# jeong0982/gkr

Hardware: AMD Instinct MI355X
Metric: BN254-Fr sumcheck field-ops/sec @ 2^20 vars (higher is better)
Workload: dtype u32x8

## Files before the change

gkr_amd/csrc/kernels.h:

```cpp
#pragma once
#include <hip/hip_runtime.h>
#include <stddef.h>
#include <stdint.h>

#include "fr32.h"

namespace gkr {

constexpr uint32_t kMaxBlocksPerTable = 2048;
constexpr uint32_t kMaxLayerBlocks = 2048;

struct MlePartial {
    Acc<9> lo, hi;
    uint32_t dep, pad;
};

struct LayerBatch {
    uint32_t batch;
    uint32_t pstride;
    size_t tstride, wstride;
};
inline LayerBatch single_layer() { return LayerBatch{1u, 0u, 0, 0}; }

struct LayerPartial {
    Acc<9> c0, g1, c2;
    uint32_t pad;
};

struct MleHostRec {
    Fr c0, c1;
    uint32_t dep, seq;
    uint32_t pad[14];
};
struct LayerHostRec {
    Fr c0, g1, c2;
    uint32_t seq;
    uint32_t pad[7];
};
static_assert(sizeof(MleHostRec) == 128 && sizeof(LayerHostRec) == 128, "hand-off records are one 128-byte line");

constexpr int kProdMaxJ = 3;
constexpr int kProdRecValues = 72;
struct ProdPassRec {
    Fr v[kProdRecValues];
    uint32_t seq;
    uint32_t pad[7];
};
static_assert(sizeof(ProdPassRec) == kProdRecValues * 32 + 32, "product-pass record layout");
constexpr uint32_t kProdTile = 8, kProdTileWide = 32;
inline uint32_t prod_pass_tile(uint32_t S) { return S >= 1024u ? kProdTileWide : kProdTile; }
inline uint32_t prod_pass_blocks(uint32_t S) { return S <= kProdTile ? 1u : S / prod_pass_tile(S); }
inline uint32_t prod_pass_max_blocks(uint32_t k) {
    uint32_t m = 1;
    for (uint32_t l = 0; l < k; ++l) m = prod_pass_blocks(1u << l) > m ? prod_pass_blocks(1u << l) : m;
    return m;
}
inline size_t prod_pass_scratch_values(uint32_t k) { return ((size_t)prod_pass_max_blocks(k) + 64u) * kProdRecValues; }
constexpr uint32_t kProdFuseBlocks = 64;
constexpr uint32_t kProdFoldMinM = 17;
size_t prod_fold_plan_bytes();
void launch_prod_pass(Fr* W, Fr* X, Fr* Y, uint32_t m_in, uint32_t jp, const Fr* weights, uint32_t J, Fr* partials, uint32_t wstride,
                      ProdPassRec* rec, uint32_t ticket, uint32_t batch, hipStream_t s, uint32_t* arrivals = nullptr, void* fold_plans = nullptr,
                      Fr* tail = nullptr, uint32_t tail_stride = 0);
void launch_prod_c_setup(const Fr* Wb, uint32_t jp, const Fr* weights, const Fr* A, const Fr* M, Fr* X, Fr* Y, uint32_t k, uint32_t wstride,
                         uint32_t batch, hipStream_t s);

constexpr uint32_t kSmallFoldQuarter = 2048;
void launch_mle_fold_sum_small(const Fr* src, size_t src_stride, Fr* dst, size_t dst_stride, uint32_t q, uint32_t batch,
                               const FixedMul* rtab, MleHostRec* host_rec, uint32_t ticket, hipStream_t s);
void launch_mle_round_reduce(const MlePartial* partials, uint32_t nblk, uint32_t batch, MleHostRec* host_rec,
                             uint32_t ticket, hipStream_t s);

struct MleSubPartial {
    Acc<9> sum;
    uint32_t dep, pad[2];
};
constexpr int kMlePassMaxRounds = 5;
constexpr int kMleMaxSub = 1 << kMlePassMaxRounds;
struct MleHostRecSub {
    Fr sums[kMleMaxSub];
    uint32_t dep, seq;
    uint32_t pad[14];
};
static_assert(sizeof(MleHostRecSub) == 1088, "hand-off record layout");
struct MlePublish {
    MleHostRecSub* rec = nullptr;
    uint32_t* arrivals = nullptr;
    uint32_t ticket = 0, jout = 0;
};
constexpr uint32_t kSmallPassEntries = 512;
uint32_t mle_pass_blocks(uint32_t items, uint32_t jout, uint32_t batch);
uint32_t mle_multifold_blocks(uint32_t S, uint32_t jout, uint32_t batch);
bool mle_multifold_uses_mfma(uint32_t S, uint32_t nblk);
constexpr int kMlePass0Stream = 2;
constexpr uint64_t kMlePass0DeepMinPartials = 2u * 12u * 256u * 4u;
void launch_mle_sub_sums(const Fr* tables, size_t stride, uint32_t len, uint32_t batch, uint32_t nblk, MleSubPartial* partials,
                         hipStream_t s, const MlePublish* publish = nullptr);
void launch_mle_sub_reduce(const MleSubPartial* partials, uint32_t nblk, uint32_t jout, uint32_t batch, MleHostRecSub* host_rec,
                           uint32_t ticket, hipStream_t s);
size_t mle_fold_plan_bytes();
void launch_mle_fold_plan(int jin, const Fr* weights, void* plans, uint32_t batch, hipStream_t s, uint32_t threads = 0);
void launch_mle_multifold(int jin, const Fr* src, size_t src_stride, Fr* dst, size_t dst_stride, uint32_t S, uint32_t batch,
                          uint32_t nblk, const Fr* weights, const void* plans, MleSubPartial* partials, hipStream_t s,
                          const MlePublish* publish = nullptr);
void launch_mle_pass_hash_lanes(const MleHostRecSub* rec, uint32_t count, uint32_t J, uint32_t round0, uint32_t n_out, bool final_pass,
                                bool first_pass, const Fr* cts, uint32_t* dep_last, Fr* weights, Fr* out_coeffs, uint32_t* out_len, Fr* out_r,
                                hipStream_t s);
void launch_mle_multifold_small(int jin, const Fr* src, size_t src_stride, Fr* dst, size_t dst_stride, uint32_t S, uint32_t jout,
                                uint32_t batch, const Fr* weights, MleHostRecSub* host_rec, uint32_t ticket, hipStream_t s, Fr* tail = nullptr, uint32_t tail_stride = 0,
                                uint32_t planes = 1, uint32_t plane_stride = 0);
constexpr uint32_t kMleFold2Planes = 8;
uint32_t mle_multifold2_partials(uint32_t S);
uint32_t mle_multifold2_tiles(uint32_t S);
void launch_mle_fine_sums(const MleSubPartial* partials, uint32_t nblk, const Fr* weights, uint32_t batch, MleHostRecSub* host_rec, uint32_t ticket,
                          hipStream_t s);
void launch_mle_copy_weights(const Fr* src, Fr* dst, uint32_t batch, hipStream_t s);
void launch_mle_multifold2(const Fr* src, size_t src_stride, Fr* dst, size_t dst_stride, uint32_t S, uint32_t batch, const void* plans, const Fr* w2,
                           MleSubPartial* partials, hipStream_t s);
void launch_layer_round_reduce(const LayerPartial* partials, uint32_t nblk, LayerHostRec* host_rec, uint32_t ticket,
                               LayerBatch lb, hipStream_t s);
void launch_fold_small(Fr* W, uint32_t hw, const FixedMul* rtab, LayerBatch lb, hipStream_t s);
struct GateSpan {
    uint64_t base, count;
};
uint32_t gate_lists_lds_blocks(uint64_t gates, uint32_t k);
size_t gate_lists_lds_scratch_words(uint64_t gates, uint32_t k);
inline size_t gate_list_words(uint64_t gates) { return 2 * (size_t)gates + 1; }
struct GateSegs {
    uint32_t shift = 0;
    uint32_t runs = 0;
    uint32_t run_base = 0;
    uint32_t bound = 0;
    uint32_t half_bound = 0;
    uint32_t groups = 0;
    uint32_t nb = 0;
    uint64_t packed_half = 0;
    uint32_t* words = nullptr;
    uint2* items() const { return reinterpret_cast<uint2*>(words); }
    uint32_t* order() const { return words + 2 * (size_t)bound; }
    uint32_t* bucket_begin() const { return order() + bound; }
    uint32_t* group_len() const { return bucket_begin() + 2 * (size_t)nb + 2; }
    uint32_t* group_off() const { return group_len() + 2 * (size_t)groups; }
    uint32_t* packed() const { return group_off() + 2 * (size_t)groups + 2; }
};
uint32_t gate_seg_shift(GateSpan span, uint32_t k_i, uint32_t k);
size_t gate_segs_words(GateSpan span, uint32_t k_i, uint32_t k);
size_t gate_segs_scratch_words(GateSpan span, uint32_t k_i, uint32_t k);
size_t gate_seg_partial_elems(GateSpan span, uint32_t k_i, uint32_t k);
void launch_gate_lists(GateSpan span, uint32_t k_i, uint32_t k, const uint8_t* gate_type, const uint32_t* left, const uint32_t* right,
                       uint32_t* counts, uint32_t* offsets, uint32_t* cursor, uint32_t* block_sums, uint32_t* list, uint32_t* bad,
                       uint32_t* lds_scratch, GateSegs* segs, uint32_t* seg_scratch, hipStream_t s);
struct GateSet {
    const uint32_t* offsets;
    const uint32_t* cursor;
    const uint32_t* list;
    const uint32_t* plan;
    const uint8_t* gate_type;
    const uint32_t* left;
    const uint32_t* right;
    uint64_t pad;
};
static_assert(sizeof(GateSet) == 64, "one cache line per proof");
void launch_gate_uv(GateSpan span, uint32_t k_i, uint32_t k, const uint32_t* offsets, const uint32_t* cursor, const uint32_t* list,
                    const Fr* e_hi, const Fr* e_lo_mont, uint32_t kl, const Fr* W, Fr* U, Fr* V, LayerBatch lb, const GateSegs* segs,
                    Fr* partials, hipStream_t s, const GateSet* sets = nullptr);
struct CPhaseFuse {
    const Fr* Wb = nullptr;
    const Fr* weights = nullptr;
    Fr* X = nullptr;
    Fr* Y = nullptr;
    uint32_t jp = 0;
};
bool launch_gate_rows(GateSpan span, uint32_t k_i, uint32_t k, const uint32_t* offsets, const uint32_t* cursor, const uint32_t* list,
                      const Fr* e_hi, const Fr* e_lo_mont, uint32_t kl, const Fr* eq_mont, Fr* A_row, Fr* M_row, LayerBatch lb,
                      const GateSegs* segs, Fr* partials, hipStream_t s, const CPhaseFuse* fuse = nullptr, const GateSet* sets = nullptr);
void launch_fill_table(Fr* table, size_t count, uint64_t seed, hipStream_t s);
void launch_fill_shard(Fr* shard_table, size_t count, uint32_t lp, uint32_t shard, uint64_t seed, hipStream_t s);
// ... 206 lines not shown
```

gkr_amd/csrc/kernels.hip:

```cpp
#include <hip/hip_runtime.h>
#include <stdlib.h>

#include <atomic>

#include "kernels.h"
#include "options.h"
#include "dev_util.h"
#include "gate_seg.h"
#include "mfma_fold.h"
#include "mfma_cross.h"
#include "mimc7.h"

namespace gkr {


__device__ __forceinline__ uint64_t mix64(uint64_t z) {
    z = (z ^ (z >> 30)) * 0xBF58476D1CE4E5B9ULL;
    z = (z ^ (z >> 27)) * 0x94D049BB133111EBULL;
    return z ^ (z >> 31);
}

__global__ void k_fill_table(Fr* table, size_t count, uint64_t seed) {
    for (size_t i = blockIdx.x * (size_t)blockDim.x + threadIdx.x; i < count; i += (size_t)gridDim.x * blockDim.x) {
        Fr f;
// ... 254 lines not shown
        : "v"(x.x), "v"(x.y), "v"(x.z), "v"(x.w)
        : "vcc");
}

template <int U, int PPW>
__global__ void __launch_bounds__(256) k_mle_sub_sums_stream(const Fr* __restrict__ tables, size_t table_stride, uint32_t chunk, uint32_t nblk,
                                                             MleSubPartial* __restrict__ partials) {
    static_assert(U >= 2 && (U & (U - 1)) == 0, "two sets of U / 2 loads");
    constexpr int H = U / 2;
    const uint32_t lane = threadIdx.x & 63u;
    const uint32_t wave = __builtin_amdgcn_readfirstlane(threadIdx.x >> 6);
    const uint32_t p0 = (blockIdx.x * 4u + wave) * (uint32_t)PPW;
    const uint32_t rpp = chunk / (32u * U);
    const mf_v4u* src = reinterpret_cast<const mf_v4u*>(tables + (size_t)blockIdx.y * table_stride + (size_t)p0 * chunk) + lane;
    MleSubPartial* out = partials + (size_t)blockIdx.y * nblk + p0;

    mf_v4u xa[H], xb[H];
    uint32_t acc[5] = {0u, 0u, 0u, 0u, 0u}, diff = 0u;
    auto load_set = [&](mf_v4u (&x)[H], const mf_v4u* p) {
#pragma unroll
        for (int u = 0; u < H; ++u) x[u] = __builtin_nontemporal_load(p + (size_t)u * 64u);
    };
    auto add_set = [&](const mf_v4u (&x)[H]) {
#pragma unroll
        for (int u = 0; u < H; ++u) {
            half_acc_add(acc, x[u]);
            const mf_v4u v = x[u];
            diff |= (v.x ^ (uint32_t)__builtin_amdgcn_mov_dpp((int)v.x, 0x4E, 0xF, 0xF, true)) |
                    (v.y ^ (uint32_t)__builtin_amdgcn_mov_dpp((int)v.y, 0x4E, 0xF, 0xF, true)) |
                    (v.z ^ (uint32_t)__builtin_amdgcn_mov_dpp((int)v.z, 0x4E, 0xF, 0xF, true)) |
                    (v.w ^ (uint32_t)__builtin_amdgcn_mov_dpp((int)v.w, 0x4E, 0xF, 0xF, true));
        }
    };
    auto finish = [&](MleSubPartial* p) {
        const bool odd = (lane & 1u) != 0u;
        Acc<9> s;
#pragma unroll
        for (int i = 0; i < 4; ++i) {
            s.l[i] = odd ? 0u : acc[i];
            s.l[4 + i] = odd ? acc[i] : (i == 0 ? acc[4] : 0u);
        }
        s.l[8] = odd ? acc[4] : 0u;
        s = wave_sum(s);
        const uint32_t dep = __any(diff != 0u) ? 1u : 0u;
        if (lane == 0) {
            p->sum = s;
            p->dep = dep;
        }
    };

#pragma unroll
    for (int u = 0; u < H; ++u) {
        xa[u] = __builtin_nontemporal_load(src + (size_t)u * 64u);
        __builtin_amdgcn_sched_barrier(0);
    }
#pragma unroll
    for (int u = 0; u < H; ++u) {
        xb[u] = __builtin_nontemporal_load(src + (size_t)(H + u) * 64u);
        __builtin_amdgcn_sched_barrier(0);
    }
    src += (size_t)U * 64u;
    [[maybe_unused]] uint32_t left = rpp;
    for (uint32_t r = (uint32_t)PPW * rpp - 1u; r != 0u; --r) {
        add_set(xa);
        load_set(xa, src);
        __builtin_amdgcn_sched_barrier(0);
        add_set(xb);
        load_set(xb, src + (size_t)H * 64u);
        __builtin_amdgcn_sched_barrier(0);
        src += (size_t)U * 64u;
        if constexpr (PPW > 1) {
            if (--left == 0u) {
                finish(out++);
#pragma unroll
                for (int i = 0; i < 5; ++i) acc[i] = 0u;
                diff = 0u;
                left = rpp;
            }
        }
    }
    add_set(xa);
    add_set(xb);
    finish(out);
}

template <int JIN>
__global__ void __launch_bounds__(256) k_mle_multifold(const Fr* __restrict__ src, size_t src_stride, Fr* __restrict__ dst,
                                                       size_t dst_stride, uint32_t S, const Fr* __restrict__ weights,
                                                       MleSubPartial* __restrict__ partials, MlePublish pub) {
    __shared__ Acc<9> smem[4];
    const Fr* s = src + (size_t)blockIdx.y * src_stride;
    Fr* d = dst + (size_t)blockIdx.y * dst_stride;
    const Fr* w = weights + (size_t)blockIdx.y * kMleMaxSub;
    const uint32_t chunk = S / gridDim.x;
    const uint32_t begin = blockIdx.x * chunk, end = begin + chunk;
    Acc<9> acc[1] = {acc_zero<9>()};
    for (uint32_t i = begin + threadIdx.x; i < end; i += blockDim.x) {
        const Fr y = multifold_entry<JIN>(s, S, i, w);
        store_fr(d + i, y);
        acc_add_fr(acc[0], y);
    }
    block_sum<9, 1>(acc, smem);
    if (threadIdx.x == 0) {
        MleSubPartial* p = partials + (size_t)blockIdx.y * gridDim.x + blockIdx.x;
        p->sum = acc[0];
        p->dep = 0;
    }
    if (pub.arrivals) mle_publish_from_last_block(partials, pub);
}

template <int JIN>
__global__ void __launch_bounds__(1024) k_mle_fold_plan(const Fr* __restrict__ weights, MfmaFoldPlan* __restrict__ plans) {
    __shared__ __attribute__((aligned(16))) unsigned char digits[32 * 32 * (1 << JIN)];
    mfma_plan_block<JIN>(weights + (size_t)blockIdx.x * kMleMaxSub, plans + blockIdx.x, digits);
}

template <int JIN>
__global__ void __launch_bounds__(256) k_mle_multifold_mfma(const Fr* __restrict__ src, size_t src_stride, Fr* __restrict__ dst,
                                                            size_t dst_stride, uint32_t S, const MfmaFoldPlan* __restrict__ plans,
                                                            MleSubPartial* __restrict__ partials, MlePublish pub) {
    __shared__ Acc<9> smem[4];
    __shared__ __attribute__((aligned(16))) unsigned char digits[JIN > 2 ? 32 * 32 * (1 << JIN) : 16];
    const Fr* s = src + (size_t)blockIdx.y * src_stride;
    Fr* d = dst + (size_t)blockIdx.y * dst_stride;
    const uint32_t chunk = S / gridDim.x;
    const uint32_t begin = blockIdx.x * chunk;
    Acc<9> acc[1] = {acc_zero<9>()};
    mfma_multifold_block<JIN>(s, d, S, plans + blockIdx.y, begin, begin + chunk, blockIdx.x * 5u + blockIdx.y * 3u, acc[0], digits);
    block_sum<9, 1>(acc, smem);
    if (threadIdx.x == 0) {
        MleSubPartial* p = partials + (size_t)blockIdx.y * gridDim.x + blockIdx.x;
        p->sum = acc[0];
        p->dep = 0;
    }
    if (pub.arrivals) mle_publish_from_last_block(partials, pub);
}


__global__ void __launch_bounds__(256) k_mle_fine_sums(const MleSubPartial* __restrict__ partials, uint32_t nblk, const Fr* __restrict__ weights,
                                                       MleHostRecSub* __restrict__ host_rec, uint32_t ticket) {
    __shared__ Fr s_w[kMleMaxSub];
    __shared__ Fr s_p[kMleMaxSub][8];
    const uint32_t t = threadIdx.x, q = t >> 5, c = t & 31u, run = nblk >> 10;
    const MleSubPartial* p = partials + (size_t)blockIdx.x * nblk;
    s_w[t >> 3].l[t & 7u] = reinterpret_cast<const uint32_t*>(weights + (size_t)blockIdx.x * kMleMaxSub)[t];
    static_assert(kMleMaxSub * 8 == 256, "one word of the weights per thread");
    __syncthreads();
    Lazy17 dot = lazy_zero();
    for (uint32_t k = 0; k < 4u; ++k) {
        const uint32_t b = q + 8u * k;
        Acc<10> f = acc_zero<10>();
        for (uint32_t i = 0; i < run; ++i) acc_add_acc(f, p[(size_t)(b * 32u + c) * run + i].sum);
        lazy_mac_v(dot, acc_reduce(f), s_w[b]);
    }
    s_p[c][q] = lazy_reduce(dot);
    __syncthreads();
    MleHostRecSub* r = host_rec + blockIdx.x;
    if (t < kMleMaxSub) {
        Acc<9> tot = acc_zero<9>();
        for (uint32_t k = 0; k < 8u; ++k) acc_add_fr(tot, s_p[t][k]);
        r->sums[t] = acc_reduce(tot);
    }
    __syncthreads();
    if (t == 0) __hip_atomic_store(&r->seq, ticket, __ATOMIC_RELEASE, __HIP_MEMORY_SCOPE_SYSTEM);
}

// ... 1848 lines not shown
    static std::atomic<uint64_t> attr_set{0};
    int dev = 0;
    (void)hipGetDevice(&dev);
    if (LDS_T && !((attr_set.load(std::memory_order_relaxed) >> (dev & 63)) & 1u)) {
        if (hipFuncSetAttribute(reinterpret_cast<const void*>(&k_seg_pass<ROWS, LDS_T>), hipFuncAttributeMaxDynamicSharedMemorySize, 160 * 1024) != hipSuccess) {
            (void)hipGetLastError();
            launch_seg_pass_t<ROWS, false>(g, k, e_lo_mont, T, X, Y, lb, s);
            return;
        }
        attr_set.fetch_or((uint64_t)1 << (dev & 63), std::memory_order_relaxed);
    }
    const uint32_t blocks = LDS_T ? device_cus() : 4 * device_cus();
    hipLaunchKernelGGL((k_seg_pass<ROWS, LDS_T>), dim3(blocks, lb.batch), dim3(LDS_T ? 1024 : 256), lds, s, g.items(), g.order(), g.bucket_begin(),
                       g.nb, g.groups, g.group_len(), g.group_off(), g.packed(), e_lo_mont, g.shift, T, tlen,
                       (uint32_t)lb.wstride, X, Y, g.half_bound);
}
static void launch_seg_pass(bool rows, const GateSegs& g, uint32_t k, const Fr* e_lo_mont, const Fr* T, Fr* X, Fr* Y, LayerBatch lb, hipStream_t s) {
    const bool no_lds = opt(OPT_gate_segments_no_lds) != 0;
    const bool lds_t = !no_lds && ((size_t)sizeof(Fr) << k) <= 128 * 1024;
    if (rows)
        lds_t ? launch_seg_pass_t<true, true>(g, k, e_lo_mont, T, X, Y, lb, s) : launch_seg_pass_t<true, false>(g, k, e_lo_mont, T, X, Y, lb, s);
    else
        lds_t ? launch_seg_pass_t<false, true>(g, k, e_lo_mont, T, X, Y, lb, s) : launch_seg_pass_t<false, false>(g, k, e_lo_mont, T, X, Y, lb, s);
}

void launch_exclusive_scan(const uint32_t* in, uint32_t* out, uint32_t* block_sums, size_t n, hipStream_t s) {
    const uint32_t sblocks = (uint32_t)((n + kScanPerBlock - 1) / kScanPerBlock);
    hipLaunchKernelGGL(k_scan_blocks, dim3(sblocks), dim3(256), 0, s, in, out, block_sums, n);
    hipLaunchKernelGGL(k_scan_sums, dim3(1), dim3(1024), 0, s, block_sums, sblocks);
    hipLaunchKernelGGL(k_scan_add, dim3(sblocks), dim3(256), 0, s, out, (uint32_t*)nullptr, block_sums, n);
}

static uint32_t bucket_threads(uint64_t gates, uint32_t k) { return (gates >> k) > 64u ? 256u : 64u; }

void launch_gate_uv(GateSpan span, uint32_t k_i, uint32_t k, const uint32_t* offsets, const uint32_t* cursor, const uint32_t* list,
                    const Fr* e_hi, const Fr* e_lo_mont, uint32_t kl, const Fr* W, Fr* U, Fr* V, LayerBatch lb, const GateSegs* segs,
                    Fr* partials, hipStream_t s, const GateSet* sets) {
    if (segs && segs->shift && partials && !sets) {
        Fr *X = partials, *Y = partials + (size_t)segs->half_bound * lb.batch;
        launch_seg_pass(false, *segs, k, e_lo_mont, W, X, Y, lb, s);
        hipLaunchKernelGGL(k_seg_combine, dim3(((1u << k) + 1u) / 2u, lb.batch), dim3(64), 0, s, segs->items(), segs->bucket_begin(), 0u, 1u << k, X, Y,
                           segs->half_bound, e_hi, k_i - segs->shift, segs->run_base, U, V, (uint32_t)lb.wstride, CPhaseFuse{});
        return;
    }
    hipLaunchKernelGGL(k_gate_uv, dim3(1u << k, lb.batch), dim3(bucket_threads(span.count, k)), 0, s, offsets, cursor, list,
                       list + gate_list_words(span.count), e_hi, e_lo_mont, kl, k_i - kl, W, U, V, (uint32_t)lb.wstride, (uint32_t)span.base, sets);
}

bool launch_gate_rows(GateSpan span, uint32_t k_i, uint32_t k, const uint32_t* offsets, const uint32_t* cursor, const uint32_t* list,
                      const Fr* e_hi, const Fr* e_lo_mont, uint32_t kl, const Fr* eq_mont, Fr* A_row, Fr* M_row, LayerBatch lb,
                      const GateSegs* segs, Fr* partials, hipStream_t s, const CPhaseFuse* fuse, const GateSet* sets) {
    if (segs && segs->shift && partials && !sets) {
        Fr *X = partials, *Y = partials + (size_t)segs->half_bound * lb.batch;
        launch_seg_pass(true, *segs, k, e_lo_mont, eq_mont, X, Y, lb, s);
        hipLaunchKernelGGL(k_seg_combine, dim3(((1u << k) + 1u) / 2u, lb.batch), dim3(64), 0, s, segs->items(), segs->bucket_begin(), 1u << k, 1u << k, X, Y,
                           segs->half_bound, e_hi, k_i - segs->shift, segs->run_base, A_row, M_row, (uint32_t)lb.wstride, fuse ? *fuse : CPhaseFuse{});
        return fuse != nullptr;
    }
    hipLaunchKernelGGL(k_gate_rows, dim3(1u << k, lb.batch), dim3(bucket_threads(span.count, k)), 0, s, offsets, cursor, list,
                       list + gate_list_words(span.count), e_hi, e_lo_mont, kl, k_i - kl, eq_mont, A_row, M_row, k, (uint32_t)lb.wstride,
                       (uint32_t)span.base, sets);
    return false;
}

void launch_predicate_normalise(const unsigned long long* wide, Fr* out, size_t cells, hipStream_t s) {
    hipLaunchKernelGGL(k_predicate_normalise, dim3(blocks_for(cells, 4096)), dim3(256), 0, s, wide, out, cells);
}

void launch_mle_fold_sum_small(const Fr* src, size_t src_stride, Fr* dst, size_t dst_stride, uint32_t q, uint32_t batch,
                               const FixedMul* rtab, MleHostRec* host_rec, uint32_t ticket, hipStream_t s) {
    hipLaunchKernelGGL(k_mle_fold_sum_small, dim3(batch), dim3(256), 0, s, src, src_stride, dst, dst_stride, q, rtab,
                       host_rec, ticket);
}

uint32_t mle_pass_blocks(uint32_t items, uint32_t jout, uint32_t batch) {
    uint32_t want = mle_blocks_per_table(items, batch);
    uint32_t b = 1u << jout;
    while (b < want && b * 2 <= items && b * 2 <= kMaxBlocksPerTable) b <<= 1;
    if (b > items) b = items;
    return b;
}

static int mle_sub_sums_stream_form(uint32_t len, uint32_t batch, uint32_t nblk, bool publishes) {
    const long long want = opt(OPT_pass0_stream) == 1 || opt(OPT_pass0_stream) == 2 ? opt(OPT_pass0_stream) : kMlePass0Stream;
    if (want != 2 || publishes || nblk == 0 || len % nblk != 0) return 0;
    const uint32_t chunk = len / nblk;
    if (chunk % 512u == 0 && nblk % 8u == 0 && (uint64_t)batch * nblk >= kMlePass0DeepMinPartials) return 2;
    return chunk % 256u == 0 && nblk % 4u == 0 ? 1 : 0;
}

void launch_mle_sub_sums(const Fr* tables, size_t stride, uint32_t len, uint32_t batch, uint32_t nblk, MleSubPartial* partials,
                         hipStream_t s, const MlePublish* publish) {
    const int form = mle_sub_sums_stream_form(len, batch, nblk, publish != nullptr);
    if (form == 2)
        hipLaunchKernelGGL((k_mle_sub_sums_stream<16, 2>), dim3(nblk / 8u, batch), dim3(256), 0, s, tables, stride, len / nblk, nblk, partials);
    else if (form == 1)
        hipLaunchKernelGGL((k_mle_sub_sums_stream<8, 1>), dim3(nblk / 4u, batch), dim3(256), 0, s, tables, stride, len / nblk, nblk, partials);
    else
        hipLaunchKernelGGL(k_mle_sub_sums, dim3(nblk, batch), dim3(256), 0, s, tables, stride, len, partials, publish ? *publish : MlePublish{});
}

void launch_mle_sub_reduce(const MleSubPartial* partials, uint32_t nblk, uint32_t jout, uint32_t batch, MleHostRecSub* host_rec,
                           uint32_t ticket, hipStream_t s) {
    hipLaunchKernelGGL(k_mle_sub_reduce, dim3(batch), dim3(512), 0, s, partials, nblk, jout, host_rec, ticket);
}

bool mle_multifold_uses_mfma(uint32_t S, uint32_t nblk) {
    const bool off = opt(OPT_no_mfma_fold) != 0;
    return !off && nblk > 0 && S % nblk == 0 && (S / nblk) % 64u == 0;
}

size_t mle_fold_plan_bytes() { return sizeof(MfmaFoldPlan); }

void launch_mle_fold_plan(int jin, const Fr* weights, void* plans, uint32_t batch, hipStream_t s, uint32_t threads) {
    MfmaFoldPlan* pl = static_cast<MfmaFoldPlan*>(plans);
    if (jin == 1)
        hipLaunchKernelGGL(k_mle_fold_plan<1>, dim3(batch), dim3(64), 0, s, weights, pl);
    else if (jin == 2)
        hipLaunchKernelGGL(k_mle_fold_plan<2>, dim3(batch), dim3(128), 0, s, weights, pl);
    else if (jin == 3)
        hipLaunchKernelGGL(k_mle_fold_plan<3>, dim3(batch), dim3(256), 0, s, weights, pl);
    else if (jin == 4)
        hipLaunchKernelGGL(k_mle_fold_plan<4>, dim3(batch), dim3(512), 0, s, weights, pl);
    else
        hipLaunchKernelGGL(k_mle_fold_plan<5>, dim3(batch), dim3(threads ? threads : 1024u), 0, s, weights, pl);
}

void launch_mle_multifold(int jin, const Fr* src, size_t src_stride, Fr* dst, size_t dst_stride, uint32_t S, uint32_t batch,
                          uint32_t nblk, const Fr* weights, const void* plans, MleSubPartial* partials, hipStream_t s,
                          const MlePublish* publish) {
    dim3 grid(nblk, batch);
    const MlePublish pub = publish ? *publish : MlePublish{};
    if (mle_multifold_uses_mfma(S, nblk)) {
        const MfmaFoldPlan* pl = static_cast<const MfmaFoldPlan*>(plans);
        if (jin == 1)
            hipLaunchKernelGGL(k_mle_multifold_mfma<1>, grid, dim3(256), 0, s, src, src_stride, dst, dst_stride, S, pl, partials, pub);
        else if (jin == 2)
            hipLaunchKernelGGL(k_mle_multifold_mfma<2>, grid, dim3(256), 0, s, src, src_stride, dst, dst_stride, S, pl, partials, pub);
        else if (jin == 3)
            hipLaunchKernelGGL(k_mle_multifold_mfma<3>, grid, dim3(256), 0, s, src, src_stride, dst, dst_stride, S, pl, partials, pub);
        else if (jin == 4)
            hipLaunchKernelGGL(k_mle_multifold_mfma<4>, grid, dim3(256), 0, s, src, src_stride, dst, dst_stride, S, pl, partials, pub);
        else
            hipLaunchKernelGGL(k_mle_multifold_mfma<5>, grid, dim3(256), 0, s, src, src_stride, dst, dst_stride, S, pl, partials, pub);
        return;
    }
    if (jin == 1)
        hipLaunchKernelGGL(k_mle_multifold<1>, grid, dim3(256), 0, s, src, src_stride, dst, dst_stride, S, weights, partials, pub);
    else if (jin == 2)
        hipLaunchKernelGGL(k_mle_multifold<2>, grid, dim3(256), 0, s, src, src_stride, dst, dst_stride, S, weights, partials, pub);
    else
        hipLaunchKernelGGL(k_mle_multifold<3>, grid, dim3(256), 0, s, src, src_stride, dst, dst_stride, S, weights, partials, pub);
}

uint32_t mle_multifold_blocks(uint32_t S, uint32_t jout, uint32_t batch) {
    const bool off = opt(OPT_no_mfma_fold) != 0;
    if (off) return mle_pass_blocks(S, jout, batch);
    const uint32_t target = opt(OPT_fold_blocks) > 0 ? (uint32_t)opt(OPT_fold_blocks) : 65536u;
    const uint32_t mc = (uint32_t)opt(OPT_fold_min_chunk);
    const uint32_t min_chunk = mc >= 64u && (mc & (mc - 1u)) == 0 ? mc : 256u;
    uint32_t b = 1u << jout;
    while ((uint64_t)b * batch < target && S / (2u * b) >= min_chunk && 2u * b <= kMaxBlocksPerTable) b <<= 1;
    if (b > S) b = S;
    return b;
}

void launch_mle_multifold_small(int jin, const Fr* src, size_t src_stride, Fr* dst, size_t dst_stride, uint32_t S, uint32_t jout,
                                uint32_t batch, const Fr* weights, MleHostRecSub* host_rec, uint32_t ticket, hipStream_t s, Fr* tail, uint32_t tail_stride,
                                uint32_t planes, uint32_t plane_stride) {
    dim3 grid(batch);
    const uint32_t threads = planes > 1 && S <= 256u ? 256u : 1024u;
    if (jin == 0)
        hipLaunchKernelGGL(k_mle_sums_small, grid, dim3(256), 0, s, src, src_stride, S, jout, host_rec, ticket);
    else
        hipLaunchKernelGGL(k_mle_multifold_small, grid, dim3(threads), threads * sizeof(Fr), s, src, src_stride, dst, dst_stride, S, (uint32_t)jin, jout, weights,
                           host_rec, ticket, tail, tail_stride, planes, plane_stride);
}
// ... 39 lines not shown
```

gkr_amd/csrc/options.h:

```cpp
#pragma once
#include <stdlib.h>
#include <string.h>

namespace gkr {

#define GKR_CONTEXT_OPTIONS(X)                                                                                                       \
                                                                  \
    X(rounds_per_pass, "rounds_per_pass", "GKR_ROUNDS_PER_PASS", 0, "rounds a pass of the plain sumcheck covers (0: 5; 3 without the MFMA fold)") \
    X(no_mfma_fold, "no_mfma_fold", "GKR_NO_MFMA_FOLD", 0, "fold passes on v_mad_u64_u32 instead of int8 MFMA")                      \
    X(first_fold_levels, "first_fold_levels", "GKR_FIRST_FOLD_LEVELS", 0, "variables the first fold of a host-hashed 2^18 .. 2^24-point sumcheck binds: 1 five, 2 ten in the one read (0: the default, capi_internal.h kMleFirstFoldLevels)") \
    X(pass0_stream, "pass0_stream", "GKR_PASS0_STREAM", 0, "pass 0 of a streaming launch of the plain sumcheck: 1 k_mle_sub_sums (a block per partial), 2 its pipelined form (a wave per one or two partials, 16-byte loads kept in flight) where it applies (0: the default, kernels.h kMlePass0Stream)") \
    X(fold2_tiles, "fold2_tiles", "GKR_FOLD2_TILES", 0, "64-entry tiles a block of the two-level first fold takes: k forces min(k, 2^(n-16)), a power of two (0: one, which is fastest where measured)") \
    X(no_fused_reduce, "no_fused_reduce", "GKR_NO_FUSED_REDUCE", 0, "latency-bound passes publish through k_mle_sub_reduce instead of from their last block") \
    X(hash_chunk, "hash_chunk", "GKR_HASH_CHUNK", 0, "8 or 16: sumchecks per host hash call (0: 16 when host threads are scarce)")    \
    X(device_hash_percent, "device_hash_percent", "GKR_DEVICE_HASH_PERCENT", 0, "share of a batch of >= 64 plain sumchecks hashed on the device (0..90)") \
    X(group_size, "group_size", "GKR_GROUP_SIZE", 0, "sumchecks per scheduling group of a batch (0: groups of ~4 GiB of tables)")     \
    X(pass_queue_depth, "pass_queue_depth", "GKR_PASS_QUEUE_DEPTH", 0, "groups whose pass 0 is queued up front (0: two)")           \
    X(no_late_stream, "no_late_stream", "GKR_NO_LATE_STREAM", 0, "a group's small late passes stay on the main stream")              \
    X(plan_main, "plan_main", "GKR_PLAN_MAIN", 0, "the fold plan (digit matrix) on the main stream instead of the side stream")       \
    X(mle_per_round, "mle_per_round", "GKR_MLE_PER_ROUND", 0, "one variable per pass (the first schedule; what the device transcript uses)") \
    X(fold_blocks, "fold_blocks", "GKR_FOLD_BLOCKS", 0, "target block count of a fold pass (0: 65536)")                              \
    X(fold_min_chunk, "fold_min_chunk", "GKR_FOLD_MIN_CHUNK", 0, "smallest chunk of entries per fold block (0: 256)")                \
    X(items_per_block, "items_per_block", "GKR_ITEMS_PER_BLOCK", 0, "entries per block of the first pass (0: 1024)")                 \
                                                                \
    X(predicate_atomics, "predicate_atomics", "GKR_PREDICATE_ATOMICS", 0, "dense predicate tables by widened-atomic scatter instead of the counting sort") \
    X(gate_groups_min_k, "gate_groups_min_k", "GKR_GATE_GROUPS_MIN_K", -1, "smallest k_next whose layers take the wide layers' item passes (-1: 13)") \
    X(no_fused_publish, "no_fused_publish", "GKR_NO_FUSED_PUBLISH", 0, "product passes publish through a second launch instead of from their last block") \
    X(gate_sort_global, "gate_sort_global", "GKR_GATE_SORT_GLOBAL", 0, "the gate lists' counting sort with global atomics where the LDS sort applies") \
    X(gate_segments_off, "gate_segments_off", "GKR_GATE_SEGMENTS_OFF", 0, "bucket kernels instead of the segment passes on large layers") \
    X(gate_segments_min_log2, "gate_segments_min_log2", "GKR_GATE_SEGMENTS_MIN_LOG2", 22, "smallest layer (log2 gates) that takes the segment passes") \
    X(gate_segment_log2, "gate_segment_log2", "GKR_GATE_SEGMENT_LOG2", 0, "log2 of the segments' mean length (0: 4)")              \
    X(gate_segments_no_lds, "gate_segments_no_lds", "GKR_GATE_SEGMENTS_NO_LDS", 0, "the segment pass gathers its table from L2 instead of LDS") \
    X(no_mfma_cross, "no_mfma_cross", "GKR_NO_MFMA_CROSS", 0, "wide layers' product passes over tables of 2^15 entries and more on v_mad_u64_u32 instead of int8 MFMA") \
    X(prod_cross_min_log2, "prod_cross_min_log2", "GKR_PROD_CROSS_MIN_LOG2", 0, "smallest tables (log2 entries, at least 13) whose cross sums of a product pass run on the matrix cores (0: 15)") \
    X(prod_fold_min_log2, "prod_fold_min_log2", "GKR_PROD_FOLD_MIN_LOG2", 0, "smallest tables (log2 entries) whose pending fold of a product pass runs on the matrix cores (0: 17)") \
    X(host_tail_log2, "host_tail_log2", "GKR_HOST_TAIL_LOG2", 0, "a phase's product passes over tables of 2^this entries and fewer run on the host (0: 6; -1: none; at most 12)") \
    X(host_tail_max_batch, "host_tail_max_batch", "GKR_HOST_TAIL_MAX_BATCH", 0, "largest batch (proofs advancing together) whose small product passes run on the host (0: 8)") \
    X(line_stepwise, "line_stepwise", "GKR_LINE_STEPWISE", 0, "q_i in its wide-layer form (one launch per variable) at every width")  \
    X(layer_no_fused, "layer_no_fused", "GKR_LAYER_NO_FUSED", 0, "device transcript: separate fold and sum kernels in the b-phase")   \
                                  \
    X(no_circuit_cache, "no_circuit_cache", "GKR_NO_CIRCUIT_CACHE", 0, "do not keep proven circuits' gate arrays and lists on the device between calls") \
    X(prove_many_pieces, "prove_many_pieces", "GKR_PROVE_MANY_PIECES", 0, "gkr_prove_many: cut the costliest items in two until there are this many")      \
    X(prove_many_lockstep, "prove_many_lockstep", "GKR_PROVE_MANY_LOCKSTEP", 1, "gkr_prove_many: items whose circuits share a k list advance in lockstep, one launch per pass for the group (0: one chain per item)") \
    X(lockstep_max_proofs, "lockstep_max_proofs", "GKR_LOCKSTEP_MAX_PROOFS", 0, "most proofs one lockstep group may hold (0: 32 -- beyond that independent chains overlap better)") \
                                                                \
    X(verify_workspace_mb, "verify_workspace_mb", "GKR_VERIFY_WORKSPACE_MB", 0, "gkr_verify_prepared / gkr_sumcheck_mle_verify*: MiB of device workspace a chunk of proofs may take (0: 2048; a chunk is never less than one proof)") \
    X(verify_device_hash_min, "verify_device_hash_min", "GKR_VERIFY_DEVICE_HASH_MIN", 0, "gkr_verify_prepared / gkr_sumcheck_mle_verify*: smallest number of round vectors in a chunk whose challenge hashes run on the device (0: the measured default, capi_verify.hip kVerifyDeviceHashMinRows; -1: never, the host threads hash; 1: always)") \
                         \
    X(mle_eval_mfma_min_n, "mle_eval_mfma_min_n", "GKR_MLE_EVAL_MFMA_MIN_N", 0, "gkr_mle_eval_batch_device / gkr_sumcheck_mle_verify*: smallest n whose tables are evaluated by the streaming matrix-core kernel (0: the default, kernels.h kMleEvalMfmaMinN; never below 11, where the kernel starts to apply; above 24: the one-block kernel up to n = 24, its largest)")

enum OptionId : int {
#define GKR_OPT_ENUM(id, name, env, def, doc) OPT_##id,
    GKR_CONTEXT_OPTIONS(GKR_OPT_ENUM)
#undef GKR_OPT_ENUM
        OPT_COUNT
};

struct OptionInfo {
    const char* name;
    const char* env;
    long long def;
    const char* doc;
};

inline const OptionInfo* option_table() {
    static const OptionInfo table[OPT_COUNT] = {
#define GKR_OPT_ROW(id, name, env, def, doc) {name, env, def, doc},
        GKR_CONTEXT_OPTIONS(GKR_OPT_ROW)
#undef GKR_OPT_ROW
    };
    return table;
}

struct Options {
    long long v[OPT_COUNT];
    static Options from_environment() {
        Options o;
        const OptionInfo* t = option_table();
        for (int i = 0; i < OPT_COUNT; ++i) {
            o.v[i] = t[i].def;
            if (const char* e = getenv(t[i].env)) {
                char* end = nullptr;
                const long long val = strtoll(e, &end, 0);
                o.v[i] = end != e ? val : 1;
            }
        }
        return o;
    }
};

inline int option_index(const char* name) {
    if (!name) return -1;
    const OptionInfo* t = option_table();
    for (int i = 0; i < OPT_COUNT; ++i)
// ... 36 lines not shown
```

Baseline: 494.4 billion.

## Add rolling single-buffer pass-0 sum kernel with XCD-contiguous block remap

Adds a new pass-0 sub-sum kernel that keeps one rolling buffer of sixteen nontemporal 16-byte loads in flight per wave, one partial per wave, and reissues each slot's load as soon as it is consumed. It also remaps workgroup IDs so that each XCD processes a contiguous eighth of the launch, which should improve locality across the per-XCD caches. This form becomes the default where the deep-stream path applies. The aim is steadier memory-level parallelism and better cache behaviour for this bandwidth-bound reduction, at the cost of launching twice as many blocks and adding index-remapping arithmetic.

```diff
diff --git a/gkr_amd/csrc/kernels.h b/gkr_amd/csrc/kernels.h
--- a/gkr_amd/csrc/kernels.h
+++ b/gkr_amd/csrc/kernels.h
@@ -92,7 +92,7 @@
 uint32_t mle_pass_blocks(uint32_t items, uint32_t jout, uint32_t batch);
 uint32_t mle_multifold_blocks(uint32_t S, uint32_t jout, uint32_t batch);
 bool mle_multifold_uses_mfma(uint32_t S, uint32_t nblk);
-constexpr int kMlePass0Stream = 2;
+constexpr int kMlePass0Stream = 3;
 constexpr uint64_t kMlePass0DeepMinPartials = 2u * 12u * 256u * 4u;
 void launch_mle_sub_sums(const Fr* tables, size_t stride, uint32_t len, uint32_t batch, uint32_t nblk, MleSubPartial* partials,
                          hipStream_t s, const MlePublish* publish = nullptr);
diff --git a/gkr_amd/csrc/kernels.hip b/gkr_amd/csrc/kernels.hip
--- a/gkr_amd/csrc/kernels.hip
+++ b/gkr_amd/csrc/kernels.hip
@@ -360,6 +360,86 @@
     add_set(xa);
     add_set(xb);
     finish(out);
+}
+
+__device__ __forceinline__ void half_piece_eat(uint32_t (&acc)[5], uint32_t& diff, const mf_v4u& v) {
+    half_acc_add(acc, v);
+    diff |= (v.x ^ (uint32_t)__builtin_amdgcn_mov_dpp((int)v.x, 0x4E, 0xF, 0xF, true)) |
+            (v.y ^ (uint32_t)__builtin_amdgcn_mov_dpp((int)v.y, 0x4E, 0xF, 0xF, true)) |
+            (v.z ^ (uint32_t)__builtin_amdgcn_mov_dpp((int)v.z, 0x4E, 0xF, 0xF, true)) |
+            (v.w ^ (uint32_t)__builtin_amdgcn_mov_dpp((int)v.w, 0x4E, 0xF, 0xF, true));
+}
+
+__device__ __forceinline__ void half_sums_finish(const uint32_t (&acc)[5], uint32_t diff, uint32_t lane, MleSubPartial* p) {
+    const bool odd = (lane & 1u) != 0u;
+    Acc<9> s;
+#pragma unroll
+    for (int i = 0; i < 4; ++i) {
+        s.l[i] = odd ? 0u : acc[i];
+        s.l[4 + i] = odd ? acc[i] : (i == 0 ? acc[4] : 0u);
+    }
+    s.l[8] = odd ? acc[4] : 0u;
+    s = wave_sum(s);
+    const uint32_t dep = __any(diff != 0u) ? 1u : 0u;
+    if (lane == 0) {
+        p->sum = s;
+        p->dep = dep;
+    }
+}
+
+template <int U, int PPW, bool XCD>
+__global__ void __launch_bounds__(256) k_mle_sub_sums_roll(const Fr* __restrict__ tables, size_t table_stride, uint32_t chunk, uint32_t nblk,
+                                                           MleSubPartial* __restrict__ partials) {
+    static_assert(U >= 4 && U % 4 == 0, "the pointer moves once per four pieces");
+    const uint32_t lane = threadIdx.x & 63u;
+    const uint32_t wave = __builtin_amdgcn_readfirstlane(threadIdx.x >> 6);
+    uint32_t bx = blockIdx.x, by = blockIdx.y;
+    if constexpr (XCD) {
+        const uint32_t nwg = gridDim.x * gridDim.y, L = by * gridDim.x + bx, q = nwg >> 3, r = nwg & 7u, run = L & 7u;
+        const uint32_t M = (run < r ? run * (q + 1u) : r * (q + 1u) + (run - r) * q) + (L >> 3);
+        by = M / gridDim.x;
+        bx = M - by * gridDim.x;
+    }
+    const uint32_t p0 = (bx * (blockDim.x >> 6) + wave) * (uint32_t)PPW;
+    const uint32_t rpp = chunk / (32u * U);
+    MleSubPartial* out = partials + (size_t)by * nblk + p0;
+    const uint32_t voff = lane * 16u;
+    uint64_t next = reinterpret_cast<uint64_t>(tables + (size_t)by * table_stride + (size_t)p0 * chunk);
+
+    mf_v4u x[U];
+    uint32_t acc[5] = {0u, 0u, 0u, 0u, 0u}, diff = 0u;
+    auto load_step = [&](int u) {
+        asm volatile("" : "+s"(next));
+        typedef const __attribute__((address_space(1))) mf_v4u* GlobalPiece;
+        x[u] = __builtin_nontemporal_load(reinterpret_cast<GlobalPiece>(next + voff) + 64 * (u & 3));
+        if ((u & 3) == 3) next += 4096u;
+    };
+#pragma unroll
+    for (int u = 0; u < U; ++u) {
+        load_step(u);
+        __builtin_amdgcn_sched_barrier(0);
+    }
+    [[maybe_unused]] uint32_t left = rpp;
+    for (uint32_t r = (uint32_t)PPW * rpp - 1u; r != 0u; --r) {
+#pragma unroll
+        for (int u = 0; u < U; ++u) {
+            half_piece_eat(acc, diff, x[u]);
+            load_step(u);
+            __builtin_amdgcn_sched_barrier(0);
+        }
+        if constexpr (PPW > 1) {
+            if (--left == 0u) {
+                half_sums_finish(acc, diff, lane, out++);
+#pragma unroll
+                for (int i = 0; i < 5; ++i) acc[i] = 0u;
+                diff = 0u;
+                left = rpp;
+            }
+        }
+    }
+#pragma unroll
+    for (int u = 0; u < U; ++u) half_piece_eat(acc, diff, x[u]);
+    half_sums_finish(acc, diff, lane, out);
 }
 
 template <int JIN>
@@ -2374,17 +2454,20 @@
 }
 
 static int mle_sub_sums_stream_form(uint32_t len, uint32_t batch, uint32_t nblk, bool publishes) {
-    const long long want = opt(OPT_pass0_stream) == 1 || opt(OPT_pass0_stream) == 2 ? opt(OPT_pass0_stream) : kMlePass0Stream;
-    if (want != 2 || publishes || nblk == 0 || len % nblk != 0) return 0;
+    const long long o = opt(OPT_pass0_stream);
+    const long long want = o >= 1 && o <= 3 ? o : kMlePass0Stream;
+    if (want < 2 || publishes || nblk == 0 || len % nblk != 0) return 0;
     const uint32_t chunk = len / nblk;
-    if (chunk % 512u == 0 && nblk % 8u == 0 && (uint64_t)batch * nblk >= kMlePass0DeepMinPartials) return 2;
+    if (chunk % 512u == 0 && nblk % 8u == 0 && (uint64_t)batch * nblk >= kMlePass0DeepMinPartials) return want == 3 ? 3 : 2;
     return chunk % 256u == 0 && nblk % 4u == 0 ? 1 : 0;
 }
 
 void launch_mle_sub_sums(const Fr* tables, size_t stride, uint32_t len, uint32_t batch, uint32_t nblk, MleSubPartial* partials,
                          hipStream_t s, const MlePublish* publish) {
     const int form = mle_sub_sums_stream_form(len, batch, nblk, publish != nullptr);
-    if (form == 2)
+    if (form == 3)
+        hipLaunchKernelGGL((k_mle_sub_sums_roll<16, 1, true>), dim3(nblk / 4u, batch), dim3(256), 0, s, tables, stride, len / nblk, nblk, partials);
+    else if (form == 2)
         hipLaunchKernelGGL((k_mle_sub_sums_stream<16, 2>), dim3(nblk / 8u, batch), dim3(256), 0, s, tables, stride, len / nblk, nblk, partials);
     else if (form == 1)
         hipLaunchKernelGGL((k_mle_sub_sums_stream<8, 1>), dim3(nblk / 4u, batch), dim3(256), 0, s, tables, stride, len / nblk, nblk, partials);
diff --git a/gkr_amd/csrc/options.h b/gkr_amd/csrc/options.h
--- a/gkr_amd/csrc/options.h
+++ b/gkr_amd/csrc/options.h
@@ -9,7 +9,7 @@
     X(rounds_per_pass, "rounds_per_pass", "GKR_ROUNDS_PER_PASS", 0, "rounds a pass of the plain sumcheck covers (0: 5; 3 without the MFMA fold)") \
     X(no_mfma_fold, "no_mfma_fold", "GKR_NO_MFMA_FOLD", 0, "fold passes on v_mad_u64_u32 instead of int8 MFMA")                      \
     X(first_fold_levels, "first_fold_levels", "GKR_FIRST_FOLD_LEVELS", 0, "variables the first fold of a host-hashed 2^18 .. 2^24-point sumcheck binds: 1 five, 2 ten in the one read (0: the default, capi_internal.h kMleFirstFoldLevels)") \
-    X(pass0_stream, "pass0_stream", "GKR_PASS0_STREAM", 0, "pass 0 of a streaming launch of the plain sumcheck: 1 k_mle_sub_sums (a block per partial), 2 its pipelined form (a wave per one or two partials, 16-byte loads kept in flight) where it applies (0: the default, kernels.h kMlePass0Stream)") \
+    X(pass0_stream, "pass0_stream", "GKR_PASS0_STREAM", 0, "pass 0 of a streaming launch of the plain sumcheck: 1 k_mle_sub_sums (a block per partial), 2 its pipelined form (a wave per one or two partials, 16-byte loads kept in flight in two sets) where it applies, 3 as 2 with the rolling form (a wave per partial, ONE buffer of sixteen loads, every XCD on a contiguous eighth of the launch) in place of the form of two partials per wave (0: the default, kernels.h kMlePass0Stream)") \
     X(fold2_tiles, "fold2_tiles", "GKR_FOLD2_TILES", 0, "64-entry tiles a block of the two-level first fold takes: k forces min(k, 2^(n-16)), a power of two (0: one, which is fastest where measured)") \
     X(no_fused_reduce, "no_fused_reduce", "GKR_NO_FUSED_REDUCE", 0, "latency-bound passes publish through k_mle_sub_reduce instead of from their last block") \
     X(hash_chunk, "hash_chunk", "GKR_HASH_CHUNK", 0, "8 or 16: sumchecks per host hash call (0: 16 when host threads are scarce)")    \
```

After: 501.2 billion (median of 6 runs). 1.4% higher.
